# caidj0/Raytracer-2025

Measured on NVIDIA B200. Metric: paths_per_sec, higher is better.
Workload: dtype f64

## Files before the change

raytracer-2025_b200/csrc/api.cu:

```cuda
#include <cuda_runtime.h>

#include <algorithm>
#include <cstdio>
#include <cstdlib>
#include <cstring>
#include <memory>
#include <mutex>
#include <new>
#include <string>
#include <thread>
#include <vector>

#include "compile.h"
#include "kernels.h"
#include "rt2025.h"

using namespace rt;

namespace {

thread_local std::string g_err;

int set_err(int code, const std::string& msg) {
    g_err = msg;
// ... 247 lines not shown
        if (rc != RT_OK) return set_err(rc, err);
        if (!device_build) {
            rc = check_device(opts ? opts->device : -1, device, sms);
            if (rc != RT_OK) return rc;
        }
        {
            const size_t budget = EXTEND_SMEM_MAX / EXTEND_MIN_BLOCKS - 1024;
            const size_t stacks = (size_t)std::min<uint32_t>(std::max(cs.bvh_depth + 2, 3 * cs.bvh4_depth + 2), TRAVERSAL_STACK) * EXTEND_BLOCK * sizeof(uint32_t) + EXTEND_RAY_SMEM_BYTES;
            if (!cs.nodes4.empty() && cs.nodes.size() * sizeof(Node) <= 2 * budget && stacks + cs.nodes4.size() * sizeof(Node4) > budget &&
                !getenv("RT2025_WIDE_BVH")) {
                RawVec<Node4>().swap(cs.nodes4);
                cs.world_root4 = INVALID_REF;
            }
        }
        s = new rt_scene();
        s->device = device;
        s->sm_count = sms;
        SceneView& v = s->view;
        keep_pool_memory(device);
        {
            cudaStream_t st = cudaStreamPerThread;
            Arena a;
            a.reserve(cs.nodes4), a.reserve(cs.nodes), a.reserve(cs.geom), a.reserve(cs.meta), a.reserve(cs.xforms), a.reserve(cs.materials), a.reserve(cs.textures);
            a.reserve(cs.images), a.reserve(cs.texels), a.reserve(cs.perlins), a.reserve(cs.media), a.reserve(cs.lights), a.reserve(cs.remaps), a.reserve(cs.walk_lean);
            a.allocate(st);
            s->arena = a.base;
            v.nodes4 = a.put(cs.nodes4, st), v.world_root4 = cs.world_root4;
            v.nodes = a.put(cs.nodes, st), v.geom = a.put(cs.geom, st), v.meta = a.put(cs.meta, st), v.xforms = a.put(cs.xforms, st);
            v.materials = a.put(cs.materials, st), v.textures = a.put(cs.textures, st), v.images = a.put(cs.images, st);
            v.texels = a.put(cs.texels, st), v.perlins = a.put(cs.perlins, st), v.media = a.put(cs.media, st);
            v.lights = a.put(cs.lights, st), v.remaps = a.put(cs.remaps, st), v.walk_lean = a.put(cs.walk_lean, st);
            CU(cudaStreamSynchronize(st));
        }
        v.world_root = cs.world_root;
        v.n_media = (uint32_t)cs.media.size();
        v.n_xforms = (uint32_t)cs.xforms.size();
        v.kinds = (cs.n_spheres && !cs.n_planars) ? 1u : ((cs.n_planars && !cs.n_spheres) ? 2u : 0u);
        v.n_lights = (uint32_t)cs.lights.size();
        v.n_prims = (uint32_t)cs.geom.size();
        s->ranks = cs.ranks;
        for (auto& m : cs.media) s->generic_media |= m.single_sphere == RT_NONE;
        v.media_xform = 0;
        for (auto& m : cs.media)
            if (m.xform != RT_NONE || (m.single_sphere != RT_NONE && cs.meta[m.single_sphere].xform != RT_NONE)) v.media_xform = 1;
        for (auto& m : cs.materials) s->class_mask |= 1u << m.shade_class;
        for (auto& t : cs.textures) s->black_texture.push_back(t.kind == RT_TEX_SOLID && t.color[0] == 0.0 && t.color[1] == 0.0 && t.color[2] == 0.0);
        uint32_t n_thick = 0, n_thick_entries = 0;
        for (auto& m : cs.media)
            if (m.flags & MEDIUM_THICK) s->class_mask |= 1u << SC_WALK, n_thick++, n_thick_entries += m.n_entry != MEDIUM_NO_ENTRIES;
        v.walk_entries_only = n_thick == 1 && n_thick_entries == 1;
        s->lights_flat = 1;
        for (auto& l : cs.lights)
            if (l.weight != 1.0 / (double)cs.lights.size()) s->lights_flat = 0;
        rt_scene_info& i = s->info;
// ... 362 lines not shown
                    cudaEventDestroy(ws.events.back());
                    ws.events.pop_back();
                }
            }
        }
        launch_finalize(W.accum, n_px_img * 3, cam->pixel_sample_scale, d_accum, o.accum_type == RT_ACCUM_F64, grid_g, st);
        launches += 1;
        CU(cudaEventRecord(ev[1], st));
        CU(cudaEventSynchronize(ev[1]));
        CU(cudaGetLastError());
        if (stats) {
            float ms = 0;
            CU(cudaEventElapsedTime(&ms, ev[0], ev[1]));
            const Counters zero{};
            const Counters& c = final_counters ? *final_counters : zero;
            stats->paths = nominal_paths;
            stats->segments = total_paths ? c.segments : 0;
            stats->node_visits = total_paths ? c.node_visits : 0;
            stats->prim_tests = total_paths ? c.prim_tests : 0;
            stats->errors = total_paths ? c.errors : 0;
            stats->iterations = total_paths ? c.iterations : 0;
            stats->reserved[0] = total_paths ? c.walk_segments : 0;
            stats->reserved[1] = total_paths ? c.walk_lean_segments : 0;
            stats->kernel_launches = launches;
            stats->ms_total = ms;
            stats->ms_raygen = ms_gen, stats->ms_extend = ms_ext, stats->ms_shade = ms_shd;
            stats->ms_other = ms_med;
        }
    } catch (const CudaFail& f) {
        rc = set_err(RT_ERR_CUDA, f.what);
    }
    for (auto& e : ev)
        if (e) cudaEventDestroy(e);
    return rc;
}

int rt_render(const rt_scene* s, const rt_camera* cam, const rt_render_opts* opts, void* accum, rt_stats* stats) {
    if (!s || !cam || !accum) return set_err(RT_ERR_INVALID, "null argument");
    const size_t elem = (opts && opts->accum_type == RT_ACCUM_F64) ? 8 : 4;
    const size_t bytes = (size_t)cam->image_width * cam->image_height * 3 * elem;
    void* d = nullptr;
    int rc = RT_OK;
    DeviceGuard guard;
    try {
        CU(cudaSetDevice(s->device));
        scratch_alloc(&d, bytes);
// ... 264 lines not shown
```

raytracer-2025_b200/csrc/compile.cpp:

```cpp
#include "compile.h"

#include <omp.h>

#include <memory>
#include <parallel/algorithm>

#include <chrono>
#include <cstdio>
#include <cstdlib>

#include <vector_functions.h>

#include <algorithm>
#include <cmath>
#include <cstring>
#include <limits>

namespace rt {

namespace {

struct V3 {
    double x, y, z;
};
// ... 962 lines not shown
            med.flags = 0;
            if (!all_spheres || !(min_depth > 0.0)) continue;
            const double radius = std::fabs(out.geom[med.single_sphere].d[6]);
            if (radius * std::fabs(1.0 / med.neg_inv_density) >= min_depth) med.flags |= MEDIUM_THICK;
        }
        for (size_t m = 0; m < out.media.size(); m++) {
            Medium& med = out.media[m];
            med.n_entry = MEDIUM_NO_ENTRIES;
            if (!(med.flags & MEDIUM_THICK) || getenv("RT2025_WALK_NO_ENTRIES")) continue;
            GroupBox b = group_boxes[group_of_medium[m]];
            for (int k = 0; k < 3; k++) {
                const float pad = 1e-4f * std::max(1.0f, std::max(std::fabs(b.lo[k]), std::fabs(b.hi[k])));
                b.lo[k] -= pad, b.hi[k] += pad;
            }
            uint32_t n = 0;
            const double* g = out.geom[med.single_sphere].d;
            const bool plain = med.xform == RT_NONE && out.meta[med.single_sphere].xform == RT_NONE && g[3] == 0.0 && g[4] == 0.0 && g[5] == 0.0;
            const double ball[4] = {g[0], g[1], g[2], std::fabs(g[6]) * (1.0 + 1e-4) + 1e-4};
            if (overlapping_leaves(b, plain ? ball : nullptr, out.world_root, med.entry, n)) med.n_entry = n;
            if (timer.on) fprintf(stderr, "[rt2025 compile] medium %zu is optically thick: %d entry leaves\n", m, (int)med.n_entry);
        }
        walk_lean();
        if (timer.on) fprintf(stderr, "[rt2025 compile] random walk: %s\n", out.walk_lean.empty() ? "generic" : (out.walk_lean[0].shell != RT_NONE ? "lean, shell" : "lean"));
        return RT_OK;
    }

    void walk_lean() {
        out.walk_lean.clear();
        const size_t n_media = out.media.size(), n_lights = out.lights.size();
        if (n_media > WALK_LEAN_MEDIA || n_lights > WALK_LEAN_LIGHTS) return;
        WalkLean L;
        std::memset(&L, 0, sizeof(L));
        L.n_media = (uint32_t)n_media, L.n_lights = (uint32_t)n_lights, L.thick = RT_NONE, L.shell = RT_NONE;
        for (size_t m = 0; m < n_media; m++) {
            const Medium& med = out.media[m];
            if (med.single_sphere == RT_NONE || med.xform != RT_NONE || out.meta[med.single_sphere].xform != RT_NONE) return;
            if (med.flags & MEDIUM_THICK) {
                if (L.thick != RT_NONE || med.n_entry == MEDIUM_NO_ENTRIES) return;
                L.thick = (uint32_t)m;
            }
            std::memcpy(L.sphere[m], out.geom[med.single_sphere].d, 7 * sizeof(double));
            L.neg_inv_density[m] = med.neg_inv_density;
            L.rank[m] = med.rank, L.medium_index[m] = med.medium_index;
        }
        if (L.thick == RT_NONE) return;
        const Medium& thick = out.media[L.thick];
        const Material& iso = out.materials[thick.material];
        if (iso.kind != RT_MAT_ISOTROPIC || iso.tex >= out.textures.size() || out.textures[iso.tex].kind != RT_TEX_SOLID) return;
        for (int k = 0; k < 3; k++) L.axp[k] = (1.0 / (4.0 * 3.14159265358979323846264338327950288)) * out.textures[iso.tex].color[k];
        for (size_t i = 0; i < n_lights; i++) {
            const Light& l = out.lights[i];
            if (l.xform != RT_NONE || l.weight != 1.0 / (double)n_lights) return;
            L.lights[i] = l;
        }
        for (uint32_t e = 0; e < thick.n_entry; e++) {
            const uint32_t first = (thick.entry[e] & ~LEAF_FLAG) >> 3, count = (thick.entry[e] & 7u) + 1;
            for (uint32_t pi = first; pi < first + count; pi++) {
                const PrimMeta& pm = out.meta[pi];
                if (L.n_prims == WALK_LEAN_PRIMS || pm.xform != RT_NONE) return;
                const uint32_t k = L.n_prims++;
                L.prim[k] = out.geom[pi];
                L.prim_kind[k] = pm.kind_mat >> 30, L.prim_rank[k] = pm.rank;
                if (L.shell == RT_NONE && L.prim_kind[k] == PRIM_SPHERE && std::memcmp(out.geom[pi].d, L.sphere[L.thick], 7 * sizeof(double)) == 0) L.shell = k;
            }
        }
        out.walk_lean.push_back(L);
    }
};

}

int compile_scene(const rt_scene_desc& d, uint32_t flags, CompiledScene& out, std::string& err, WorldBuilder world_builder) {
    Compiler c{d, flags, out, err};
    c.world_builder = world_builder;
    return c.run();
}

}
```

raytracer-2025_b200/csrc/compile.h:

```cpp
#pragma once
#include <memory>
#include <string>
#include <type_traits>
#include <utility>
#include <vector>

#include <vector_types.h>

#include "rt2025.h"
#include "scene_types.h"

namespace rt {

template <class T, class A = std::allocator<T>>
struct default_init_allocator : A {
    using A::A;
    template <class U>
    struct rebind {
        using other = default_init_allocator<U, typename std::allocator_traits<A>::template rebind_alloc<U>>;
    };
    template <class U>
    void construct(U* p) noexcept(std::is_nothrow_default_constructible<U>::value) {
        ::new (static_cast<void*>(p)) U;
    }
// ... 3 lines not shown
    }
};
template <class T>
using RawVec = std::vector<T, default_init_allocator<T>>;

struct CompiledScene {
    RawVec<Node> nodes;
    RawVec<Node4> nodes4;
    uint32_t world_root4 = INVALID_REF;
    uint32_t bvh4_depth = 0;
    RawVec<PrimGeom> geom;
    RawVec<PrimMeta> meta;
    std::vector<Xform> xforms;
    std::vector<Material> materials;
    std::vector<Texture> textures;
    std::vector<Image> images;
    std::vector<float4> texels;
    std::vector<Perlin> perlins;
    std::vector<Medium> media;
    std::vector<Light> lights;
    std::vector<Remap> remaps;
    std::vector<uint32_t> ranks;
    std::vector<WalkLean> walk_lean;
    uint32_t world_root = INVALID_REF;
    uint32_t bvh_depth = 0;
    uint32_t media_bvh_depth = 0;
    uint32_t n_spheres = 0, n_planars = 0;
};

struct BuildBox;
using WorldBuilder = bool (*)(const RawVec<BuildBox>& boxes, uint32_t first_prim_base, RawVec<Node>& nodes,
                              RawVec<uint32_t>& order, uint32_t& depth_out, uint32_t& root_out);

int compile_scene(const rt_scene_desc& d, uint32_t flags, CompiledScene& out, std::string& err, WorldBuilder world_builder = nullptr);

uint32_t collapse_bvh4(const RawVec<Node>& nodes, uint32_t root, RawVec<Node4>& out, uint32_t& depth_out);

struct BuildBox {
    float lo[3], hi[3];
};
uint32_t build_bvh(const RawVec<BuildBox>& boxes, uint32_t first_prim_base, RawVec<Node>& nodes,
                   RawVec<uint32_t>& order, uint32_t& depth_out);
bool build_bvh_device(const RawVec<BuildBox>& boxes, uint32_t first_prim_base, RawVec<Node>& nodes, RawVec<uint32_t>& order,
                      uint32_t& depth_out, uint32_t& root_out);

}
// ... 1 lines not shown
```

raytracer-2025_b200/csrc/kernels.cu:

```cuda
#include <cuda_runtime.h>
#include <stdint.h>

#include <algorithm>

#include "kernels.h"
#include "shade.cuh"

namespace rt {

struct RayArrayIO {
    const SceneView& sv;
    const rt_ray* __restrict__ rays;
    rt_hit* __restrict__ out;
    double tmin, tmax;
    __device__ __forceinline__ double t_min() const { return tmin; }
    __device__ __forceinline__ bool load(uint32_t i, RayD& r, double& t1, uint32_t& prim0, uint32_t& rank0) const {
        const double* rp = reinterpret_cast<const double*>(rays + i);
        r.o = D3{rp[0], rp[1], rp[2]};
        r.d = D3{rp[3], rp[4], rp[5]};
        r.time = rp[6];
        t1 = tmax;
        prim0 = 0xFFFFFFFFu, rank0 = 0xFFFFFFFFu;
        return true;
    }
// ... 469 lines not shown
        const uint32_t local = queue_reserve(cntb, q);
        __syncthreads();
        if (threadIdx.x < SC_COUNT) {
            const uint32_t c = cntb[threadIdx.x];
            if (c) s_base[threadIdx.x] = atomicAdd(&W.counters->n_shade[threadIdx.x], c);
            s_cnt[(it & 1) ^ 1][threadIdx.x] = 0;
        }
        __syncthreads();
        if (q >= 0) W.q_shade[q][s_base[q] + local] = j;
    }
}

__device__ __forceinline__ void contribute(const RenderParams& P, const WavefrontState& W, uint32_t pixel, D3 c) {
    if (isnan(c.x) || isnan(c.y) || isnan(c.z)) {
        atomicAdd(&W.counters->errors, 1ull);
        return;
    }
    double* a = W.accum + (size_t)pixel * 3;
    if (c.x != 0.0) atomicAdd(a + 0, c.x);
    if (c.y != 0.0) atomicAdd(a + 1, c.y);
    if (c.z != 0.0) atomicAdd(a + 2, c.z);
}

template <uint32_t CLS>
__device__ __forceinline__ bool shade_one(const SceneView& sv, const RenderParams& P, const WavefrontState& W, const RayD& r, D3 beta, uint32_t pixel,
                                          uint32_t sidx, uint32_t segment, double t, uint32_t prim, uint32_t kind, RayD& nr, D3& nbeta) {
    constexpr bool GENERIC = CLS == SC_OTHER;
    constexpr bool DO_MISS = CLS == SC_MISS;
    constexpr bool DO_MEDIUM = GENERIC || CLS == SC_ISOTROPIC;
    constexpr bool DO_EMIT = GENERIC || CLS == SC_EMISSIVE || CLS == SC_DISNEY;
    constexpr bool DO_PDF = GENERIC || CLS == SC_DIFFUSE || CLS == SC_TEXTURED || CLS == SC_ISOTROPIC || CLS == SC_DISNEY;
    constexpr bool DO_REMAP = GENERIC || CLS == SC_DISNEY;
    constexpr bool DO_METAL = GENERIC || CLS == SC_METAL;
    constexpr bool DO_DIELECTRIC = GENERIC || CLS == SC_DIELECTRIC;
            bool alive = false, error = false;
            nr = r;
            nbeta = beta;

            if (DO_MISS || (GENERIC && kind == HIT_MISS)) {
                D3 bg;
                if (background_value(sv, P.cam.background_tex, r.d, bg))
                    contribute(P, W, pixel, beta * bg);
                else
                    error = true;
            } else {
                HitInfo h;
                bool hit_ok = true;
                if (DO_MEDIUM && kind == HIT_MEDIUM) {
                    const Medium& med = sv.media[prim];
// ... 82 lines not shown
                        }
                        case RT_MAT_TRANSPARENT:
                            alive = GENERIC;
                            break;
                        case RT_MAT_PORTAL: {
                            if (!GENERIC) break;
                            nr.o = h.p + ld3(M.v);
                            double qw = M.v[3], qx = M.v[4], qy = M.v[5], qz = M.v[6];
                            double aw = qw * 0.0 - qx * r.d.x - qy * r.d.y - qz * r.d.z;
                            double ax = qw * r.d.x + qx * 0.0 + qy * r.d.z - qz * r.d.y;
                            double ay = qw * r.d.y - qx * r.d.z + qy * 0.0 + qz * r.d.x;
                            double az = qw * r.d.z + qx * r.d.y - qy * r.d.x + qz * 0.0;
                            double cx = -qx, cy = -qy, cz = -qz;
                            nr.d.x = aw * cx + ax * qw + ay * cz - az * cy;
                            nr.d.y = aw * cy - ax * cz + ay * qw + az * cx;
                            nr.d.z = aw * cz + ax * cy - ay * cx + az * qw;
                            nbeta = beta * ld3(M.color);
                            alive = true;
                            break;
                        }
                        case RT_MAT_LAMBERTIAN: {
                            const bool iso = CLS == SC_ISOTROPIC || (GENERIC && M.kind == RT_MAT_ISOTROPIC);
                            const bool dis = CLS == SC_DISNEY || (GENERIC && M.kind == RT_MAT_DISNEY);
                            D3 albedo = (M.kind == RT_MAT_EMPTY || dis) ? D3{0.75, 0.75, 0.75} : texture_value(sv, M.tex, h.u, h.v, h.p);
                            ONB uvw;
                            if (!iso && !make_onb(h.normal, uvw)) {
                                error = true;
                                break;
                            }
                            disney::Params DP;
                            D3 v_out_l = D3{0.0, 1.0, 0.0};
                            if (dis) {
                                DP.base_color = M.tex == RT_NONE ? ld3(M.color) : texture_value(sv, M.tex, h.u, h.v, h.p);
                                DP.roughness = M.v[RT_DISNEY_ROUGHNESS], DP.anisotropic = M.v[RT_DISNEY_ANISOTROPIC], DP.sheen = M.v[RT_DISNEY_SHEEN];
                                DP.sheen_tint = M.v[RT_DISNEY_SHEEN_TINT], DP.clearcoat = M.v[RT_DISNEY_CLEARCOAT];
                                DP.clearcoat_gloss = M.v[RT_DISNEY_CLEARCOAT_GLOSS], DP.specular_tint = M.v[RT_DISNEY_SPECULAR_TINT];
                                DP.metallic = M.v[RT_DISNEY_METALLIC], DP.ior = M.v[RT_DISNEY_IOR], DP.flatness = M.v[RT_DISNEY_FLATNESS];
                                DP.spec_trans = M.v[RT_DISNEY_SPEC_TRANS], DP.diff_trans = M.v[RT_DISNEY_DIFF_TRANS], DP.thin = M.v[RT_DISNEY_THIN] != 0.0;
                                D3 vo;
                                if (!unit_vector(-r.d, vo)) {
                                    error = true;
                                    break;
                                }
                                v_out_l = D3{dot(vo, uvw.u), dot(vo, uvw.v), dot(vo, uvw.w)};
                            }
                            Rand2 pick = philox_pair(P.seed, pixel, sidx, segment, RT_SLOT_MIXTURE);
                            Rand2 dx = philox_pair(P.seed, pixel, sidx, segment, RT_SLOT_DIRECTION);
                            D3 gen = D3{0.0, 0.0, 0.0};
                            const bool have_lights = sv.n_lights > 0;
                            int stop = 0;
                            if (have_lights && !(pick.a < 0.5)) {
                                if (!lights_random(sv, h.p, pick.b, dx.a, dx.b, gen)) stop = 1;
                            } else if (dis) {
                                Rand2 dpick = philox_pair(P.seed, pixel, sidx, segment, RT_SLOT_DISNEY);
                                D3 v_in_l;
                                bool derr = false;
                                if (!disney::generate_local(DP, v_out_l, h.front_face, dpick, dx, v_in_l, derr))
                                    stop = derr ? 1 : 2;
                                else if (!unit_vector(onb_to_world(uvw, v_in_l), gen))
                                    stop = 1;
                            } else {
                                gen = iso ? random_unit_vector(dx.a, dx.b) : onb_to_world(uvw, random_cosine_direction(dx.a, dx.b));
                            }
                            D3 axp = D3{0.0, 0.0, 0.0};
                            double value0 = 0.0;
                            if (!stop) {
                                if (iso) {
                                    value0 = 1.0 / (4.0 * RT_PI);
                                    axp = albedo / (4.0 * RT_PI);
                                } else {
                                    D3 ud;
                                    if (!unit_vector(gen, ud)) {
                                        stop = 1;
                                    } else if (dis) {
                                        D3 v_in_l = D3{dot(ud, uvw.u), dot(ud, uvw.v), dot(ud, uvw.w)};
                                        bool derr = false;
                                        disney::evaluate_disney(DP, v_out_l, v_in_l, h.front_face, axp, value0, derr);
                                        if (derr) stop = 1;
                                    } else {
                                        double cosine_theta = dot(ud, uvw.v);
                                        value0 = rmax(0.0, cosine_theta / RT_PI);
                                        axp = albedo * rmax(cosine_theta, 0.0) / RT_PI;
                                    }
                                }
                            }
                            double pdf_val = value0;
                            if (!stop && have_lights) {
                                double value1 = lights_pdf_value(sv, P.lights_flat, h.p, gen);
                                if (isnan(value1) || (value0 == 0.0 && value1 == 0.0))
                                    stop = 1;
                                else
                                    pdf_val = value0 * 0.5 + value1 * 0.5;
                            }
                            if (!stop && pdf_val == 0.0) stop = 1;
                            if (!stop) {
                                nr.d = gen;
                                nbeta = beta * (axp / pdf_val);
                                alive = true;
                            }
                            if (stop == 1) error = true;
                            break;
                        }
                        default: break;
                    }
                }
            }
            if (error) {
                atomicAdd(&W.counters->errors, 1ull);
                alive = false;
            }
            if (alive && (segment + 1 >= P.cam.max_depth || (nbeta.x == 0.0 && nbeta.y == 0.0 && nbeta.z == 0.0))) alive = false;
            return alive;
}

template <uint32_t CLS>
__global__ void __launch_bounds__(SHADE_BLOCK, ((RT_SHADE_3BLOCK_MASK >> CLS) & 1u) ? 3 : RT_SHADE_MIN_BLOCKS) k_shade(SceneView sv, RenderParams P, WavefrontState W, uint32_t queue) {
    __shared__ uint32_t s_warp_count[SHADE_BLOCK / 32];
    __shared__ uint32_t s_base;
    const uint32_t n = W.counters->n_shade[queue];
    const RayRec* __restrict__ rays = W.ray_q[W.parity];
    const BetaRec* __restrict__ betas = W.beta_q[W.parity];
    for (uint32_t j0 = blockIdx.x * blockDim.x; j0 < n; j0 += gridDim.x * blockDim.x) {
        const uint32_t j = j0 + threadIdx.x;
        int q = -1;
        RayD nr;
        D3 nbeta;
        uint32_t pixel = 0, sidx = 0, segment = 0;
#if RT_SHADE_PREFETCH
        {
            const uint32_t jn = j + gridDim.x * blockDim.x;
            if (jn < n) {
                const uint32_t pn = W.q_shade[queue][jn];
                asm volatile("prefetch.global.L2 [%0];" ::"l"(rays + pn));
                asm volatile("prefetch.global.L2 [%0];" ::"l"(betas + pn));
                asm volatile("prefetch.global.L2 [%0];" ::"l"(W.hit_q + pn));
            }
        }
#endif
        if (j < n) {
            const uint32_t pos = W.q_shade[queue][j];
            RayD r;
            uint64_t ids64;
            load_ray(rays + pos, r, ids64);
            unpack_ids(ids64, pixel, sidx, segment);
            const double2* sp2 = reinterpret_cast<const double2*>(betas + pos);
            const double2 b0 = sp2[0], b1 = sp2[1];
            D3 beta = D3{b0.x, b0.y, b1.x};
            const double2 hw = *reinterpret_cast<const double2*>(W.hit_q + pos);
            const double t = hw.x;
            const uint32_t prim = (uint32_t)__double2hiint(hw.y), kind = (uint32_t)__double2loint(hw.y);
            const bool alive = shade_one<CLS>(sv, P, W, r, beta, pixel, sidx, segment, t, prim, kind, nr, nbeta);
            q = alive ? 0 : -1;
        }
        const unsigned alive_mask = __ballot_sync(0xFFFFFFFFu, q == 0);
        const uint32_t warp = threadIdx.x >> 5, lane = threadIdx.x & 31u;
        if (lane == 0) s_warp_count[warp] = __popc(alive_mask);
        __syncthreads();
        if (threadIdx.x == 0) {
            uint32_t total = 0;
#pragma unroll
            for (int w = 0; w < SHADE_BLOCK / 32; w++) total += s_warp_count[w];
            s_base = total ? atomicAdd(&W.counters->n_extend[W.parity ^ 1u], total) : 0u;
        }
        __syncthreads();
        uint32_t npos = s_base + __popc(alive_mask & ((1u << lane) - 1u));
        for (uint32_t w = 0; w < warp; w++) npos += s_warp_count[w];
        __syncthreads();
        if (q == 0) {
            store_ray(W.ray_q[W.parity ^ 1u] + npos, nr, pack_ids(pixel, sidx, segment + 1));
            store_beta(W.beta_q[W.parity ^ 1u] + npos, nbeta);
        }
    }
}

#ifndef RT_WALK_BLOCK
#define RT_WALK_BLOCK 128
#endif
constexpr int WALK_BLOCK = RT_WALK_BLOCK;
#ifndef RT_WALK_MIN_BLOCKS
#define RT_WALK_MIN_BLOCKS 4
#endif
#ifndef RT_WALK_LEAN_MIN_BLOCKS
#define RT_WALK_LEAN_MIN_BLOCKS 4
#endif

__device__ __forceinline__ bool walk_lean_segment(const SceneView& sv, const WalkLean& L, const RenderParams& P, const WavefrontState& W, const RayD& r,
                                                  D3 beta, uint32_t pixel, uint32_t sidx, uint32_t segment, double t, uint32_t max_steps,
                                                  uint32_t& steps, RayD& nr, D3& nbeta, double& tn, bool& stay) {
    stay = false;
    nr.o = r.o + t * r.d;
    nr.time = r.time;
    const Rand2 pick = philox_pair(P.seed, pixel, sidx, segment, RT_SLOT_MIXTURE);
    const Rand2 dx = philox_pair(P.seed, pixel, sidx, segment, RT_SLOT_DIRECTION);
    const uint32_t n_lights = L.n_lights;
    D3 gen = D3{0.0, 0.0, 0.0};
    bool panic = false;
    if (n_lights > 0 && !(pick.a < 0.5)) {
        uint32_t leaf = n_lights - 1;
        for (uint32_t i = 0; i < n_lights; i++)
            if (pick.b < L.lights[i].cdf) {
                leaf = i;
                break;
            }
        panic = !light_leaf_random(L.lights[leaf], nr.o, dx.a, dx.b, gen);
    } else {
        gen = random_unit_vector(dx.a, dx.b);
    }
    const double value0 = 1.0 / (4.0 * RT_PI);
    double pdf_val = value0;
    if (!panic && n_lights > 0) {
        double sum = 0.0;
        for (uint32_t i = 0; i < n_lights; i++) sum += light_leaf_pdf<true>(sv, L.lights[i], nr.o, gen);
        const double value1 = n_lights == 1 ? sum : sum / (double)n_lights;
        if (isnan(value1) || (value0 == 0.0 && value1 == 0.0))
            panic = true;
        else
            pdf_val = value0 * 0.5 + value1 * 0.5;
    }
    if (panic || pdf_val == 0.0) {
        atomicAdd(&W.counters->errors, 1ull);
        return false;
    }
    nr.d = gen;
    nbeta = beta * (ld3(L.axp) / pdf_val);
    if (segment + 1 >= P.cam.max_depth || (nbeta.x == 0.0 && nbeta.y == 0.0 && nbeta.z == 0.0)) return false;

    const uint32_t seg1 = segment + 1u, thick = L.thick;
    MediumDraws draws;
    double near_root, far_root;
    {
        const double* s = L.sphere[thick];
        double t1, t2;
        const double xi = draws.get(P.seed, pixel, sidx, seg1, L.medium_index[thick]);
        const bool inside = sphere_entry_exit_at(ld3(s), ld3(s + 3), s[6], nr, t1, t2, near_root, far_root);
        if (!inside || !medium_free_flight(t1, t2, nr, L.neg_inv_density[thick], xi, tn)) return true;
    }
    if (!(++steps < max_steps)) return true;
    const uint32_t med_rank = L.rank[thick];
    for (uint32_t m = 0; m < L.n_media; m++) {
        if (m == thick) continue;
        const double xi = draws.get(P.seed, pixel, sidx, seg1, L.medium_index[m]);
        if (RT_MEDIA_EARLY_SCREEN && free_flight_overshoots(L.neg_inv_density[m], xi, tn, nr.d)) continue;
        const double* s = L.sphere[m];
        double t1, t2, nroot, froot, tm;
        if (!sphere_entry_exit_at(ld3(s), ld3(s + 3), s[6], nr, t1, t2, nroot, froot) || !medium_free_flight(t1, t2, nr, L.neg_inv_density[m], xi, tm)) continue;
        if (tm < tn || (tm == tn && L.rank[m] < med_rank)) return true;
    }
    bool beaten = false;
// ... 297 lines not shown
        k<<<grid, MEDIA_BLOCK, 0, s>>>(sv, P, W);
        return 1;
    }
    int launches = 1;
    if (phase == 0 && sv.n_media) {
        SceneView mv = sv;
        mv.n_cached_nodes = 0;
        const size_t media_smem = generic ? (size_t)sv.media_stack_entries * MEDIA_BLOCK * sizeof(uint32_t) : 0;
        const bool xf = sv.media_xform != 0;
        if (generic) {
            auto k = count ? (xf ? k_media<true, 2, true, false> : k_media<true, 2, false, false>) : (xf ? k_media<false, 2, true, false> : k_media<false, 2, false, false>);
            k<<<grid, MEDIA_BLOCK, media_smem, s>>>(mv, P, W);
        } else {
            auto k = count ? (xf ? k_media<true, 1, true, false> : k_media<true, 1, false, false>) : (xf ? k_media<false, 1, true, false> : k_media<false, 1, false, false>);
            k<<<grid, MEDIA_BLOCK, 0, s>>>(mv, P, W);
        }
        launches++;
    }
    k_bin<<<grid, MEDIA_BLOCK, 0, s>>>(W);
    return launches;
}
template <uint32_t CLS>
static void launch_shade_cls(const SceneView& sv, const RenderParams& P, const WavefrontState& W, uint32_t queue, int grid, cudaStream_t s) {
    if ((RT_SHADE_3BLOCK_MASK >> CLS) & 1u) grid = grid / RT_SHADE_MIN_BLOCKS * 3;
    k_shade<CLS><<<grid, SHADE_BLOCK, 0, s>>>(sv, P, W, queue);
}
int launch_shade(const SceneView& sv, const RenderParams& P, const WavefrontState& W, uint32_t class_mask, int grid, cudaStream_t s,
                 const ShadeFan* fan, bool tail_follows, int walk_grid) {
    int launches = tail_follows ? 1 : 2;
    if (!P.bin_by_class) {
        launch_shade_cls<SC_MISS>(sv, P, W, SC_MISS, grid, s);
        launch_shade_cls<SC_OTHER>(sv, P, W, SC_DIFFUSE, grid, s);
        launches++;
    } else {
        const int n_side = fan ? fan->n_side : 0;
        if (n_side) {
            cudaEventRecord(fan->fork, s);
            for (int i = 0; i < n_side; i++) cudaStreamWaitEvent(fan->side[i], fan->fork, 0);
        }
        int next = 0;
        auto lane = [&]() {
            const int k = next++ % (n_side + 1);
            return k == 0 ? s : fan->side[k - 1];
        };
        if (class_mask & (1u << SC_WALK)) launch_walk(sv, P, W, walk_grid, lane()), launches++;
        if (class_mask & (1u << SC_DIFFUSE)) launch_shade_cls<SC_DIFFUSE>(sv, P, W, SC_DIFFUSE, grid, lane()), launches++;
// ... 53 lines not shown
```

raytracer-2025_b200/csrc/kernels.h:

```cpp
#pragma once
#include <cuda_runtime.h>
#include <stdint.h>

#include "rt2025.h"
#include "scene_types.h"

namespace rt {

#ifndef RT_EXTEND_BLOCK
#define RT_EXTEND_BLOCK 512
#endif
#ifndef RT_EXTEND_MIN_BLOCKS
#define RT_EXTEND_MIN_BLOCKS 1
#endif
constexpr int EXTEND_BLOCK = RT_EXTEND_BLOCK;
constexpr int EXTEND_MIN_BLOCKS = RT_EXTEND_MIN_BLOCKS;
constexpr size_t EXTEND_SMEM_MAX = 227 * 1024;
constexpr int SHADE_BLOCK = 256;
constexpr int MEDIA_BLOCK = 256;
#ifndef RT_REFILL_MIN
#define RT_REFILL_MIN 32
#endif
constexpr int REFILL_MIN = RT_REFILL_MIN;
#ifndef RT_SLAB_SIGNSEL
// ... 47 lines not shown
    double w[7];
    uint64_t ids;
};
struct alignas(16) BetaRec {
    double beta[3];
    double spare;
};
struct alignas(16) HitRec {
    double t;
    uint32_t kind, prim;
};
static_assert(sizeof(RayRec) == 64 && sizeof(BetaRec) == 32 && sizeof(HitRec) == 16, "stream record sizes");
constexpr uint32_t IDS_PIXEL_BITS = 28, IDS_SAMPLE_BITS = 24, IDS_SEGMENT_BITS = 12;

struct Counters {
    uint32_t n_extend[2];
    uint32_t n_shade[SC_COUNT];
    uint32_t n_pixels, pad;
    uint32_t n_unsampled, pad3;
    uint32_t gen_done, walk_cursor;
    unsigned long long next_path, segments, iterations, errors, node_visits, prim_tests;
    unsigned long long walk_segments;
    unsigned long long walk_lean_segments;
};

struct WavefrontState {
    RayRec* ray_q[2];
    BetaRec* beta_q[2];
    HitRec* hit_q;
    uint8_t* cls_q;
    uint32_t* q_shade[SC_COUNT];
    uint32_t* pixel_list;
    double* accum;
    Counters* counters;
    uint32_t capacity, n_pixels;
    uint64_t total_paths;
    uint32_t parity, pad;
};

struct RenderParams {
    rt_camera cam;
    uint64_t seed;
    uint32_t sample_begin, part_index, part_count;
    uint32_t lights_flat, bin_by_class;
    uint32_t walk_drain_queue, walk_drain_steps;
    uint32_t drop_misses;
// ... 30 lines not shown
```

raytracer-2025_b200/csrc/scene_types.h:

```cpp
#pragma once
#include <stdint.h>

namespace rt {

constexpr uint32_t LEAF_FLAG = 0x80000000u;
constexpr uint32_t INVALID_REF = 0x7FFFFFFFu;
constexpr int MAX_LEAF_PRIMS = 8;
constexpr int TRAVERSAL_STACK = 64;
constexpr uint32_t META_MAT_MASK = 0x03FFFFFFu;
constexpr uint32_t META_CLASS_SHIFT = 26;

struct alignas(32) Node {
    float lo0[3], hi0[3];
    float lo1[3], hi1[3];
    uint32_t child0, child1;
    uint32_t pad0, pad1;
};
static_assert(sizeof(Node) == 64, "node must be 64 bytes");

struct alignas(32) Node4 {
    float box[4][6];
    uint32_t child[4];
    uint32_t pad[4];
};
// ... 59 lines not shown
struct Medium {
    uint32_t root;
    uint32_t material;
    uint32_t object;
    uint32_t rank;
    double neg_inv_density;
    uint32_t xform;
    uint32_t medium_index;
    uint32_t single_sphere;
    uint32_t flags;
    uint32_t n_entry;
    uint32_t entry[MEDIUM_MAX_ENTRIES];
    uint32_t pad;
};
constexpr uint32_t MEDIUM_THICK = 1u;

struct Light {
    PrimGeom g;
    uint32_t kind;
    uint32_t xform;
    double weight, cdf, area;
};

constexpr uint32_t WALK_LEAN_MEDIA = 4, WALK_LEAN_LIGHTS = 4, WALK_LEAN_PRIMS = 8;
struct WalkLean {
    Light lights[WALK_LEAN_LIGHTS];
    PrimGeom prim[WALK_LEAN_PRIMS];
    double sphere[WALK_LEAN_MEDIA][8];
    double neg_inv_density[WALK_LEAN_MEDIA];
    double axp[3];
    double pad0;
    uint32_t rank[WALK_LEAN_MEDIA], medium_index[WALK_LEAN_MEDIA];
    uint32_t prim_kind[WALK_LEAN_PRIMS], prim_rank[WALK_LEAN_PRIMS];
    uint32_t n_media, thick, n_lights, n_prims;
    uint32_t shell;
    uint32_t pad1[3];
};

enum ShadeClass : uint32_t {
    SC_MISS = 0,
    SC_DIFFUSE = 1,
    SC_TEXTURED = 2,
    SC_ISOTROPIC = 3,
    SC_METAL = 4,
    SC_DIELECTRIC = 5,
    SC_EMISSIVE = 6,
    SC_DISNEY = 7,
    SC_OTHER = 8,
    SC_WALK = 9,
    SC_COUNT = 10
};

struct SceneView {
    const Node* nodes;
    const PrimGeom* geom;
    const PrimMeta* meta;
    const Xform* xforms;
    const Material* materials;
    const Texture* textures;
// ... 1 lines not shown
    const float4* texels;
    const Perlin* perlins;
    const Medium* media;
    const Light* lights;
    const Remap* remaps;
    const Node4* nodes4;
    uint32_t world_root4;
    uint32_t media_xform;
    uint32_t world_root;
    uint32_t n_media, n_lights, n_prims;
    uint32_t n_nodes;
    uint32_t n_cached_nodes;
    uint32_t stack_entries;
    uint32_t l2_window_bytes;
    uint32_t park_leaves;
    uint32_t refill_min;
    uint32_t media_stack_entries;
    uint32_t tail_stack_entries;
    uint32_t kinds;
    uint32_t n_xforms;
    uint32_t walk_entries_only;
    uint32_t fifo_slots;
    const WalkLean* walk_lean;
};

}
```

raytracer-2025_b200/csrc/shade.cuh:

```cuda
#pragma once
#include "disney.cuh"
#include "traverse.cuh"

namespace rt {

__device__ __forceinline__ int32_t as_i32_sat(double x) {
    if (isnan(x)) return 0;
    if (x >= 2147483647.0) return 2147483647;
    if (x <= -2147483648.0) return (-2147483647 - 1);
    return (int32_t)x;
}
__device__ __forceinline__ uint32_t as_u32_sat(double x) {
    if (!(x > 0.0)) return 0u;
    if (x >= 4294967295.0) return 0xFFFFFFFFu;
    return (uint32_t)x;
}

__device__ inline double perlin_noise(const Perlin* __restrict__ tab, D3 p) {
    double fx = floor(p.x), fy = floor(p.y), fz = floor(p.z);
    long long i = (long long)fx, j = (long long)fy, k = (long long)fz;
    double u = p.x - fx, v = p.y - fy, w = p.z - fz;
    double uu = u * u * (3.0 - 2.0 * u), vv = v * v * (3.0 - 2.0 * v), ww = w * w * (3.0 - 2.0 * w);
    double accum = 0.0;
#pragma unroll
// ... 240 lines not shown
    for (uint32_t i = 0; i < sv.n_lights; i++)
        if (pick < sv.lights[i].cdf) {
            leaf = i;
            break;
        }
    const Light& l = sv.lights[leaf];
    if (l.xform == RT_NONE) return light_leaf_random(l, origin, r1, r2, out);
    const Xform* x = sv.xforms + l.xform;
    const uint32_t n = x->n_chain;
    D3 origins[MAX_XFORM_CHAIN + 1];
    origins[0] = origin;
    for (uint32_t k = 0; k < n; k++) origins[k + 1] = xf_detransform(load_xform(sv.xforms + x->chain[k]), origins[k]);
    D3 dir;
    bool ok = light_leaf_random(l, origins[n], r1, r2, dir);
    for (uint32_t k = n; k-- > 0;) {
        XformParams p = load_xform(sv.xforms + x->chain[k]);
        D3 world_to = xf_transform(p, origins[k + 1] + dir);
        ok = unit_vector(world_to - origins[k], dir) && ok;
    }
    out = dir;
    return ok;
}

__device__ inline bool background_value(const SceneView& sv, uint32_t tex, D3 dir, D3& out) {
    D3 p;
    if (!unit_vector(dir, p)) return false;
    double u = 0.0, v = 0.0;
    if (texture_needs_uv(sv, tex)) {
        double theta = acos(-p.y);
        double phi = RT_PI - atan2(-p.z, p.x);
        u = phi / (2.0 * RT_PI);
        v = theta / RT_PI;
    }
    out = texture_value(sv, tex, u, v, p);
    return true;
}

__device__ inline D3 material_emitted(const SceneView& sv, uint32_t mat, const HitInfo& h) {
    D3 total = D3{0.0, 0.0, 0.0};
    uint32_t st_mat[8];
    double st_w[8];
    int sp = 0;
    st_mat[sp] = mat, st_w[sp] = 1.0, sp++;
    while (sp > 0) {
        --sp;
        uint32_t m = st_mat[sp];
// ... 20 lines not shown
```

raytracer-2025_b200/rt2025.py:

```python
import ctypes as C
import os
import subprocess

import numpy as np

PKG_DIR = os.path.dirname(os.path.abspath(__file__))
ROOT = os.path.dirname(PKG_DIR)
RT_NONE = 0xFFFFFFFF
RT_OPT_COUNT = 1
RT_OPT_STAGE_TIMES = 2
RT_ACCUM_F32 = 0
RT_ACCUM_F64 = 1
RT_BUILD_NO_REF_RANKS = 1
RT_BUILD_DEVICE_LBVH = 2

ABI_SYMBOLS = [
    "rt_scene_create", "rt_scene_destroy", "rt_closest_hit", "rt_closest_hit_device", "rt_render",
    "rt_render_device", "rt_render_rgb8", "rt_render_multi", "rt_render_multi_rgb8", "rt_tonemap", "rt_tonemap_device", "rt_scene_get_info", "rt_scene_get_ranks", "rt_last_error",
    "rt_abi_version", "rt_device_count",
]


class RtError(RuntimeError):
    pass
# ... 23 lines not shown
        ("reserved", C.c_uint32 * 4),
    ]


class rt_stats(C.Structure):
    _fields_ = [
        ("paths", C.c_uint64), ("segments", C.c_uint64), ("node_visits", C.c_uint64),
        ("prim_tests", C.c_uint64), ("errors", C.c_uint64), ("kernel_launches", C.c_uint64),
        ("ms_total", C.c_double), ("ms_raygen", C.c_double), ("ms_extend", C.c_double),
        ("ms_shade", C.c_double), ("ms_other", C.c_double), ("iterations", C.c_uint64),
        ("reserved", C.c_uint64 * 4),
    ]

    def as_dict(self):
        return {k: getattr(self, k) for k, _ in self._fields_ if k != "reserved"}

    @property
    def walk_segments(self):
        return int(self.reserved[0])

    @property
    def walk_lean_segments(self):
        return int(self.reserved[1])


class rt_scene_info(C.Structure):
    _fields_ = [
        ("n_prims", C.c_uint32), ("n_spheres", C.c_uint32), ("n_planars", C.c_uint32), ("n_nodes", C.c_uint32),
        ("n_media", C.c_uint32), ("n_lights", C.c_uint32), ("n_materials", C.c_uint32), ("n_textures", C.c_uint32),
        ("bvh_depth", C.c_uint32), ("node_bytes", C.c_uint32), ("device_bytes", C.c_uint64),
    ]


class rth_camera_params(C.Structure):
    _fields_ = [
        ("aspect_ratio", C.c_double), ("image_width", C.c_uint32), ("samples_per_pixel", C.c_uint32),
        ("max_depth", C.c_uint32), ("background_tex", C.c_uint32), ("vertical_fov_in_degrees", C.c_double),
        ("look_from", C.c_double * 3), ("look_at", C.c_double * 3), ("vec_up", C.c_double * 3),
        ("defocus_angle_in_degrees", C.c_double), ("focus_distance", C.c_double),
        ("toon_map", C.c_uint32), ("reserved", C.c_uint32),
    ]


class rt_scene_desc(C.Structure):
    _fields_ = [
        ("version", C.c_uint32), ("struct_size", C.c_uint32), ("world_root", C.c_uint32), ("lights_root", C.c_uint32),
# ... 388 lines not shown
```

Before: 1.509 billion.

## Add lean specialized shade kernels for diffuse, textured, isotropic and emissive classes

After: 1.586 billion, median of 6. 5.2% higher.

```diff
diff --git a/raytracer-2025_b200/csrc/api.cu b/raytracer-2025_b200/csrc/api.cu
--- a/raytracer-2025_b200/csrc/api.cu
+++ b/raytracer-2025_b200/csrc/api.cu
@@ -293,7 +293,7 @@
             cudaStream_t st = cudaStreamPerThread;
             Arena a;
             a.reserve(cs.nodes4), a.reserve(cs.nodes), a.reserve(cs.geom), a.reserve(cs.meta), a.reserve(cs.xforms), a.reserve(cs.materials), a.reserve(cs.textures);
-            a.reserve(cs.images), a.reserve(cs.texels), a.reserve(cs.perlins), a.reserve(cs.media), a.reserve(cs.lights), a.reserve(cs.remaps), a.reserve(cs.walk_lean);
+            a.reserve(cs.images), a.reserve(cs.texels), a.reserve(cs.perlins), a.reserve(cs.media), a.reserve(cs.lights), a.reserve(cs.remaps), a.reserve(cs.walk_lean), a.reserve(cs.shade_lean);
             a.allocate(st);
             s->arena = a.base;
             v.nodes4 = a.put(cs.nodes4, st), v.world_root4 = cs.world_root4;
@@ -301,6 +301,7 @@
             v.materials = a.put(cs.materials, st), v.textures = a.put(cs.textures, st), v.images = a.put(cs.images, st);
             v.texels = a.put(cs.texels, st), v.perlins = a.put(cs.perlins, st), v.media = a.put(cs.media, st);
             v.lights = a.put(cs.lights, st), v.remaps = a.put(cs.remaps, st), v.walk_lean = a.put(cs.walk_lean, st);
+            v.shade_lean = a.put(cs.shade_lean, st), v.shade_lean_mask = cs.shade_lean_mask;
             CU(cudaStreamSynchronize(st));
         }
         v.world_root = cs.world_root;
@@ -709,6 +710,7 @@
             stats->iterations = total_paths ? c.iterations : 0;
             stats->reserved[0] = total_paths ? c.walk_segments : 0;
             stats->reserved[1] = total_paths ? c.walk_lean_segments : 0;
+            stats->reserved[2] = total_paths ? c.shade_lean_hits : 0;
             stats->kernel_launches = launches;
             stats->ms_total = ms;
             stats->ms_raygen = ms_gen, stats->ms_extend = ms_ext, stats->ms_shade = ms_shd;
diff --git a/raytracer-2025_b200/csrc/compile.cpp b/raytracer-2025_b200/csrc/compile.cpp
--- a/raytracer-2025_b200/csrc/compile.cpp
+++ b/raytracer-2025_b200/csrc/compile.cpp
@@ -1008,16 +1008,45 @@
         }
         walk_lean();
         if (timer.on) fprintf(stderr, "[rt2025 compile] random walk: %s\n", out.walk_lean.empty() ? "generic" : (out.walk_lean[0].shell != RT_NONE ? "lean, shell" : "lean"));
+        shade_lean();
+        if (timer.on) {
+            std::string classes;
+            const std::pair<uint32_t, const char*> names[] = {{SC_DIFFUSE, " diffuse"}, {SC_TEXTURED, " textured"}, {SC_ISOTROPIC, " isotropic"}, {SC_EMISSIVE, " emissive"}};
+            for (const auto& c : names)
+                if (out.shade_lean_mask & (1u << c.first)) classes += c.second;
+            fprintf(stderr, "[rt2025 compile] shade lean:%s\n", classes.empty() ? " generic" : classes.c_str());
+        }
         return RT_OK;
+    }
+
+    bool lean_lights(LeanLights& L) const {
+        std::memset(&L, 0, sizeof(L));
+        const size_t n = out.lights.size();
+        if (n > LEAN_LIGHTS) return false;
+        for (size_t i = 0; i < n; i++) {
+            const Light& l = out.lights[i];
+            if (l.xform != RT_NONE || l.weight != 1.0 / (double)n) return false;
+            L.lights[i] = l;
+        }
+        L.n = (uint32_t)n;
+        return true;
+    }
+
+    bool isotropic_axp(uint32_t material, double* axp) const {
+        const Material& iso = out.materials[material];
+        if (iso.kind != RT_MAT_ISOTROPIC || iso.tex >= out.textures.size() || out.textures[iso.tex].kind != RT_TEX_SOLID) return false;
+        for (int k = 0; k < 3; k++) axp[k] = (1.0 / (4.0 * 3.14159265358979323846264338327950288)) * out.textures[iso.tex].color[k];
+        return true;
     }
 
     void walk_lean() {
         out.walk_lean.clear();
-        const size_t n_media = out.media.size(), n_lights = out.lights.size();
-        if (n_media > WALK_LEAN_MEDIA || n_lights > WALK_LEAN_LIGHTS) return;
+        const size_t n_media = out.media.size();
+        if (n_media > WALK_LEAN_MEDIA) return;
         WalkLean L;
         std::memset(&L, 0, sizeof(L));
-        L.n_media = (uint32_t)n_media, L.n_lights = (uint32_t)n_lights, L.thick = RT_NONE, L.shell = RT_NONE;
+        if (!lean_lights(L.lights)) return;
+        L.n_media = (uint32_t)n_media, L.thick = RT_NONE, L.shell = RT_NONE;
         for (size_t m = 0; m < n_media; m++) {
             const Medium& med = out.media[m];
             if (med.single_sphere == RT_NONE || med.xform != RT_NONE || out.meta[med.single_sphere].xform != RT_NONE) return;
@@ -1031,14 +1060,7 @@
         }
         if (L.thick == RT_NONE) return;
         const Medium& thick = out.media[L.thick];
-        const Material& iso = out.materials[thick.material];
-        if (iso.kind != RT_MAT_ISOTROPIC || iso.tex >= out.textures.size() || out.textures[iso.tex].kind != RT_TEX_SOLID) return;
-        for (int k = 0; k < 3; k++) L.axp[k] = (1.0 / (4.0 * 3.14159265358979323846264338327950288)) * out.textures[iso.tex].color[k];
-        for (size_t i = 0; i < n_lights; i++) {
-            const Light& l = out.lights[i];
-            if (l.xform != RT_NONE || l.weight != 1.0 / (double)n_lights) return;
-            L.lights[i] = l;
-        }
+        if (!isotropic_axp(thick.material, L.axp)) return;
         for (uint32_t e = 0; e < thick.n_entry; e++) {
             const uint32_t first = (thick.entry[e] & ~LEAF_FLAG) >> 3, count = (thick.entry[e] & 7u) + 1;
             for (uint32_t pi = first; pi < first + count; pi++) {
@@ -1052,6 +1074,36 @@
         }
         out.walk_lean.push_back(L);
     }
+
+    void shade_lean() {
+        out.shade_lean.clear();
+        out.shade_lean_mask = 0;
+        ShadeLean S;
+        std::memset(&S, 0, sizeof(S));
+        const bool lights = lean_lights(S.lights);
+        bool iso = lights && out.media.size() <= SHADE_LEAN_MEDIA;
+        for (size_t m = 0; iso && m < out.media.size(); m++) {
+            const Medium& med = out.media[m];
+            if (med.flags & MEDIUM_THICK) continue;
+            iso = med.xform == RT_NONE && isotropic_axp(med.material, S.axp[m]);
+        }
+        bool emissive = true;
+        for (size_t p = 0; p < out.meta.size() && (iso || emissive); p++) {
+            const PrimMeta& pm = out.meta[p];
+            const uint32_t cls = (pm.kind_mat >> META_CLASS_SHIFT) & 15u;
+            if (cls == SC_ISOTROPIC) iso = false;
+            if (cls == SC_EMISSIVE) {
+                const Material& M = out.materials[pm.kind_mat & META_MAT_MASK];
+                if (pm.xform != RT_NONE || M.kind != RT_MAT_DIFFUSE_LIGHT || M.inner != RT_NONE || M.tex >= out.textures.size() ||
+                    out.textures[M.tex].kind != RT_TEX_SOLID)
+                    emissive = false;
+            }
+        }
+        if (lights) out.shade_lean_mask |= 1u << SC_DIFFUSE | 1u << SC_TEXTURED;
+        if (iso) out.shade_lean_mask |= 1u << SC_ISOTROPIC;
+        if (emissive) out.shade_lean_mask |= 1u << SC_EMISSIVE;
+        if (out.shade_lean_mask) out.shade_lean.push_back(S);
+    }
 };
 
 }
diff --git a/raytracer-2025_b200/csrc/compile.h b/raytracer-2025_b200/csrc/compile.h
--- a/raytracer-2025_b200/csrc/compile.h
+++ b/raytracer-2025_b200/csrc/compile.h
@@ -49,6 +49,8 @@
     std::vector<Remap> remaps;
     std::vector<uint32_t> ranks;
     std::vector<WalkLean> walk_lean;
+    std::vector<ShadeLean> shade_lean;
+    uint32_t shade_lean_mask = 0;
     uint32_t world_root = INVALID_REF;
     uint32_t bvh_depth = 0;
     uint32_t media_bvh_depth = 0;
diff --git a/raytracer-2025_b200/csrc/kernels.cu b/raytracer-2025_b200/csrc/kernels.cu
--- a/raytracer-2025_b200/csrc/kernels.cu
+++ b/raytracer-2025_b200/csrc/kernels.cu
@@ -515,9 +515,11 @@
     if (c.z != 0.0) atomicAdd(a + 2, c.z);
 }
 
-template <uint32_t CLS>
+template <uint32_t CLS, bool LEAN = false>
 __device__ __forceinline__ bool shade_one(const SceneView& sv, const RenderParams& P, const WavefrontState& W, const RayD& r, D3 beta, uint32_t pixel,
-                                          uint32_t sidx, uint32_t segment, double t, uint32_t prim, uint32_t kind, RayD& nr, D3& nbeta) {
+                                          uint32_t sidx, uint32_t segment, double t, uint32_t prim, uint32_t kind, RayD& nr, D3& nbeta,
+                                          const LeanLights* LL = nullptr) {
+    static_assert(!LEAN || CLS == SC_DIFFUSE || CLS == SC_TEXTURED, "the other lean classes have their own code");
     constexpr bool GENERIC = CLS == SC_OTHER;
     constexpr bool DO_MISS = CLS == SC_MISS;
     constexpr bool DO_MEDIUM = GENERIC || CLS == SC_ISOTROPIC;
@@ -646,7 +648,9 @@
                         case RT_MAT_LAMBERTIAN: {
                             const bool iso = CLS == SC_ISOTROPIC || (GENERIC && M.kind == RT_MAT_ISOTROPIC);
                             const bool dis = CLS == SC_DISNEY || (GENERIC && M.kind == RT_MAT_DISNEY);
-                            D3 albedo = (M.kind == RT_MAT_EMPTY || dis) ? D3{0.75, 0.75, 0.75} : texture_value(sv, M.tex, h.u, h.v, h.p);
+                            D3 albedo = (M.kind == RT_MAT_EMPTY || dis)  ? D3{0.75, 0.75, 0.75}
+                                        : (LEAN && CLS == SC_DIFFUSE) ? ld3(sv.textures[M.tex].color)
+                                                                      : texture_value(sv, M.tex, h.u, h.v, h.p);
                             ONB uvw;
                             if (!iso && !make_onb(h.normal, uvw)) {
                                 error = true;
@@ -671,10 +675,10 @@
                             Rand2 pick = philox_pair(P.seed, pixel, sidx, segment, RT_SLOT_MIXTURE);
                             Rand2 dx = philox_pair(P.seed, pixel, sidx, segment, RT_SLOT_DIRECTION);
                             D3 gen = D3{0.0, 0.0, 0.0};
-                            const bool have_lights = sv.n_lights > 0;
+                            const bool have_lights = LEAN ? LL->n > 0 : sv.n_lights > 0;
                             int stop = 0;
                             if (have_lights && !(pick.a < 0.5)) {
-                                if (!lights_random(sv, h.p, pick.b, dx.a, dx.b, gen)) stop = 1;
+                                if (!(LEAN ? lean_lights_random(*LL, h.p, pick.b, dx.a, dx.b, gen) : lights_random(sv, h.p, pick.b, dx.a, dx.b, gen))) stop = 1;
                             } else if (dis) {
                                 Rand2 dpick = philox_pair(P.seed, pixel, sidx, segment, RT_SLOT_DISNEY);
                                 D3 v_in_l;
@@ -710,7 +714,7 @@
                             }
                             double pdf_val = value0;
                             if (!stop && have_lights) {
-                                double value1 = lights_pdf_value(sv, P.lights_flat, h.p, gen);
+                                double value1 = LEAN ? lean_lights_pdf(sv, *LL, h.p, gen) : lights_pdf_value(sv, P.lights_flat, h.p, gen);
                                 if (isnan(value1) || (value0 == 0.0 && value1 == 0.0))
                                     stop = 1;
                                 else
@@ -737,10 +741,59 @@
             return alive;
 }
 
-template <uint32_t CLS>
-__global__ void __launch_bounds__(SHADE_BLOCK, ((RT_SHADE_3BLOCK_MASK >> CLS) & 1u) ? 3 : RT_SHADE_MIN_BLOCKS) k_shade(SceneView sv, RenderParams P, WavefrontState W, uint32_t queue) {
+__device__ __forceinline__ bool lean_isotropic_scatter(const SceneView& sv, const LeanLights& L, D3 axp, const RenderParams& P, const WavefrontState& W,
+                                                       const RayD& r, D3 beta, uint32_t pixel, uint32_t sidx, uint32_t segment, double t, RayD& nr,
+                                                       D3& nbeta) {
+    nr.o = r.o + t * r.d;
+    nr.time = r.time;
+    const Rand2 pick = philox_pair(P.seed, pixel, sidx, segment, RT_SLOT_MIXTURE);
+    const Rand2 dx = philox_pair(P.seed, pixel, sidx, segment, RT_SLOT_DIRECTION);
+    D3 gen = D3{0.0, 0.0, 0.0};
+    bool panic = false;
+    if (L.n > 0 && !(pick.a < 0.5))
+        panic = !lean_lights_random(L, nr.o, pick.b, dx.a, dx.b, gen);
+    else
+        gen = random_unit_vector(dx.a, dx.b);
+    const double value0 = 1.0 / (4.0 * RT_PI);
+    double pdf_val = value0;
+    if (!panic && L.n > 0) {
+        const double value1 = lean_lights_pdf(sv, L, nr.o, gen);
+        if (isnan(value1) || (value0 == 0.0 && value1 == 0.0))
+            panic = true;
+        else
+            pdf_val = value0 * 0.5 + value1 * 0.5;
+    }
+    if (panic || pdf_val == 0.0) {
+        atomicAdd(&W.counters->errors, 1ull);
+        return false;
+    }
+    nr.d = gen;
+    nbeta = beta * (axp / pdf_val);
+    return !(segment + 1 >= P.cam.max_depth || (nbeta.x == 0.0 && nbeta.y == 0.0 && nbeta.z == 0.0));
+}
+
+#ifndef RT_SHADE_LEAN_BLOCKS
+#define RT_SHADE_LEAN_BLOCKS 0x3003230u
+#endif
+constexpr int shade_lean_blocks(uint32_t cls) { return (int)((RT_SHADE_LEAN_BLOCKS >> (4u * cls)) & 15u); }
+constexpr int shade_blocks(uint32_t cls, bool lean) {
+    return lean ? shade_lean_blocks(cls) : (((RT_SHADE_3BLOCK_MASK >> cls) & 1u) ? 3 : RT_SHADE_MIN_BLOCKS);
+}
+
+template <uint32_t CLS, bool LEAN = false>
+__global__ void __launch_bounds__(SHADE_BLOCK, shade_blocks(CLS, LEAN)) k_shade(SceneView sv, RenderParams P, WavefrontState W, uint32_t queue) {
+    constexpr bool EMIT_ONLY = LEAN && CLS == SC_EMISSIVE;
     __shared__ uint32_t s_warp_count[SHADE_BLOCK / 32];
     __shared__ uint32_t s_base;
+    extern __shared__ float4 s_lean[];
+    const ShadeLean& SL = *reinterpret_cast<const ShadeLean*>(s_lean);
+    if (LEAN && !EMIT_ONLY) {
+        unsigned long long* dst = reinterpret_cast<unsigned long long*>(s_lean);
+        const unsigned long long* src = reinterpret_cast<const unsigned long long*>(sv.shade_lean);
+        for (uint32_t k = threadIdx.x; k < sizeof(ShadeLean) / 8; k += SHADE_BLOCK) dst[k] = src[k];
+        __syncthreads();
+    }
+    unsigned long long lean_hits = 0;
     const uint32_t n = W.counters->n_shade[queue];
     const RayRec* __restrict__ rays = W.ray_q[W.parity];
     const BetaRec* __restrict__ betas = W.beta_q[W.parity];
@@ -761,21 +814,38 @@
             }
         }
 #endif
+        if (LEAN && threadIdx.x == 0) lean_hits += min(n - j0, (uint32_t)SHADE_BLOCK);
         if (j < n) {
             const uint32_t pos = W.q_shade[queue][j];
-            RayD r;
-            uint64_t ids64;
-            load_ray(rays + pos, r, ids64);
-            unpack_ids(ids64, pixel, sidx, segment);
-            const double2* sp2 = reinterpret_cast<const double2*>(betas + pos);
-            const double2 b0 = sp2[0], b1 = sp2[1];
-            D3 beta = D3{b0.x, b0.y, b1.x};
-            const double2 hw = *reinterpret_cast<const double2*>(W.hit_q + pos);
-            const double t = hw.x;
-            const uint32_t prim = (uint32_t)__double2hiint(hw.y), kind = (uint32_t)__double2loint(hw.y);
-            const bool alive = shade_one<CLS>(sv, P, W, r, beta, pixel, sidx, segment, t, prim, kind, nr, nbeta);
-            q = alive ? 0 : -1;
-        }
+            if constexpr (EMIT_ONLY) {
+                unpack_ids((uint64_t)__double_as_longlong(reinterpret_cast<const double2*>(rays + pos)[3].y), pixel, sidx, segment);
+                const double2* sp2 = reinterpret_cast<const double2*>(betas + pos);
+                const double2 b0 = sp2[0], b1 = sp2[1];
+                const D3 beta = D3{b0.x, b0.y, b1.x};
+                const uint32_t prim = (uint32_t)__double2hiint(reinterpret_cast<const double2*>(W.hit_q + pos)->y);
+                const uint32_t mat = sv.meta[prim].kind_mat & META_MAT_MASK;
+                const D3 e = D3{0.0, 0.0, 0.0} + 1.0 * ld3(sv.textures[sv.materials[mat].tex].color);
+                contribute(P, W, pixel, beta * e);
+            } else {
+                RayD r;
+                uint64_t ids64;
+                load_ray(rays + pos, r, ids64);
+                unpack_ids(ids64, pixel, sidx, segment);
+                const double2* sp2 = reinterpret_cast<const double2*>(betas + pos);
+                const double2 b0 = sp2[0], b1 = sp2[1];
+                D3 beta = D3{b0.x, b0.y, b1.x};
+                const double2 hw = *reinterpret_cast<const double2*>(W.hit_q + pos);
+                const double t = hw.x;
+                const uint32_t prim = (uint32_t)__double2hiint(hw.y), kind = (uint32_t)__double2loint(hw.y);
+                bool alive;
+                if constexpr (LEAN && CLS == SC_ISOTROPIC)
+                    alive = lean_isotropic_scatter(sv, SL.lights, ld3(SL.axp[prim]), P, W, r, beta, pixel, sidx, segment, t, nr, nbeta);
+                else
+                    alive = shade_one<CLS, LEAN>(sv, P, W, r, beta, pixel, sidx, segment, t, prim, kind, nr, nbeta, &SL.lights);
+                q = alive ? 0 : -1;
+            }
+        }
+        if constexpr (EMIT_ONLY) continue;
         const unsigned alive_mask = __ballot_sync(0xFFFFFFFFu, q == 0);
         const uint32_t warp = threadIdx.x >> 5, lane = threadIdx.x & 31u;
         if (lane == 0) s_warp_count[warp] = __popc(alive_mask);
@@ -790,11 +860,14 @@
         uint32_t npos = s_base + __popc(alive_mask & ((1u << lane) - 1u));
         for (uint32_t w = 0; w < warp; w++) npos += s_warp_count[w];
         __syncthreads();
-        if (q == 0) {
-            store_ray(W.ray_q[W.parity ^ 1u] + npos, nr, pack_ids(pixel, sidx, segment + 1));
-            store_beta(W.beta_q[W.parity ^ 1u] + npos, nbeta);
-        }
-    }
+        if constexpr (!EMIT_ONLY) {
+            if (q == 0) {
+                store_ray(W.ray_q[W.parity ^ 1u] + npos, nr, pack_ids(pixel, sidx, segment + 1));
+                store_beta(W.beta_q[W.parity ^ 1u] + npos, nbeta);
+            }
+        }
+    }
+    if (LEAN && lean_hits) atomicAdd(&W.counters->shade_lean_hits, lean_hits);
 }
 
 #ifndef RT_WALK_BLOCK
@@ -812,42 +885,7 @@
                                                   D3 beta, uint32_t pixel, uint32_t sidx, uint32_t segment, double t, uint32_t max_steps,
                                                   uint32_t& steps, RayD& nr, D3& nbeta, double& tn, bool& stay) {
     stay = false;
-    nr.o = r.o + t * r.d;
-    nr.time = r.time;
-    const Rand2 pick = philox_pair(P.seed, pixel, sidx, segment, RT_SLOT_MIXTURE);
-    const Rand2 dx = philox_pair(P.seed, pixel, sidx, segment, RT_SLOT_DIRECTION);
-    const uint32_t n_lights = L.n_lights;
-    D3 gen = D3{0.0, 0.0, 0.0};
-    bool panic = false;
-    if (n_lights > 0 && !(pick.a < 0.5)) {
-        uint32_t leaf = n_lights - 1;
-        for (uint32_t i = 0; i < n_lights; i++)
-            if (pick.b < L.lights[i].cdf) {
-                leaf = i;
-                break;
-            }
-        panic = !light_leaf_random(L.lights[leaf], nr.o, dx.a, dx.b, gen);
-    } else {
-        gen = random_unit_vector(dx.a, dx.b);
-    }
-    const double value0 = 1.0 / (4.0 * RT_PI);
-    double pdf_val = value0;
-    if (!panic && n_lights > 0) {
-        double sum = 0.0;
-        for (uint32_t i = 0; i < n_lights; i++) sum += light_leaf_pdf<true>(sv, L.lights[i], nr.o, gen);
-        const double value1 = n_lights == 1 ? sum : sum / (double)n_lights;
-        if (isnan(value1) || (value0 == 0.0 && value1 == 0.0))
-            panic = true;
-        else
-            pdf_val = value0 * 0.5 + value1 * 0.5;
-    }
-    if (panic || pdf_val == 0.0) {
-        atomicAdd(&W.counters->errors, 1ull);
-        return false;
-    }
-    nr.d = gen;
-    nbeta = beta * (ld3(L.axp) / pdf_val);
-    if (segment + 1 >= P.cam.max_depth || (nbeta.x == 0.0 && nbeta.y == 0.0 && nbeta.z == 0.0)) return false;
+    if (!lean_isotropic_scatter(sv, L.lights, ld3(L.axp), P, W, r, beta, pixel, sidx, segment, t, nr, nbeta)) return false;
 
     const uint32_t seg1 = segment + 1u, thick = L.thick;
     MediumDraws draws;
@@ -1191,6 +1229,13 @@
 }
 template <uint32_t CLS>
 static void launch_shade_cls(const SceneView& sv, const RenderParams& P, const WavefrontState& W, uint32_t queue, int grid, cudaStream_t s) {
+    if constexpr (CLS == SC_DIFFUSE || CLS == SC_TEXTURED || CLS == SC_ISOTROPIC || CLS == SC_EMISSIVE) {
+        if (queue == CLS && (sv.shade_lean_mask >> CLS) & 1u) {
+            static_assert(shade_lean_blocks(CLS) >= 1, "RT_SHADE_LEAN_BLOCKS: no CTA count for a lean class");
+            k_shade<CLS, true><<<grid / RT_SHADE_MIN_BLOCKS * shade_lean_blocks(CLS), SHADE_BLOCK, CLS == SC_EMISSIVE ? 0 : sizeof(ShadeLean), s>>>(sv, P, W, queue);
+            return;
+        }
+    }
     if ((RT_SHADE_3BLOCK_MASK >> CLS) & 1u) grid = grid / RT_SHADE_MIN_BLOCKS * 3;
     k_shade<CLS><<<grid, SHADE_BLOCK, 0, s>>>(sv, P, W, queue);
 }
diff --git a/raytracer-2025_b200/csrc/kernels.h b/raytracer-2025_b200/csrc/kernels.h
--- a/raytracer-2025_b200/csrc/kernels.h
+++ b/raytracer-2025_b200/csrc/kernels.h
@@ -93,6 +93,7 @@
     unsigned long long next_path, segments, iterations, errors, node_visits, prim_tests;
     unsigned long long walk_segments;
     unsigned long long walk_lean_segments;
+    unsigned long long shade_lean_hits;
 };
 
 struct WavefrontState {
diff --git a/raytracer-2025_b200/csrc/scene_types.h b/raytracer-2025_b200/csrc/scene_types.h
--- a/raytracer-2025_b200/csrc/scene_types.h
+++ b/raytracer-2025_b200/csrc/scene_types.h
@@ -105,9 +105,16 @@
     double weight, cdf, area;
 };
 
-constexpr uint32_t WALK_LEAN_MEDIA = 4, WALK_LEAN_LIGHTS = 4, WALK_LEAN_PRIMS = 8;
+constexpr uint32_t LEAN_LIGHTS = 4;
+struct LeanLights {
+    Light lights[LEAN_LIGHTS];
+    uint32_t n;
+    uint32_t pad[7];
+};
+
+constexpr uint32_t WALK_LEAN_MEDIA = 4, WALK_LEAN_PRIMS = 8;
 struct WalkLean {
-    Light lights[WALK_LEAN_LIGHTS];
+    LeanLights lights;
     PrimGeom prim[WALK_LEAN_PRIMS];
     double sphere[WALK_LEAN_MEDIA][8];
     double neg_inv_density[WALK_LEAN_MEDIA];
@@ -115,9 +122,14 @@
     double pad0;
     uint32_t rank[WALK_LEAN_MEDIA], medium_index[WALK_LEAN_MEDIA];
     uint32_t prim_kind[WALK_LEAN_PRIMS], prim_rank[WALK_LEAN_PRIMS];
-    uint32_t n_media, thick, n_lights, n_prims;
+    uint32_t n_media, thick, n_prims;
     uint32_t shell;
-    uint32_t pad1[3];
+};
+
+constexpr uint32_t SHADE_LEAN_MEDIA = 4;
+struct ShadeLean {
+    LeanLights lights;
+    double axp[SHADE_LEAN_MEDIA][4];
 };
 
 enum ShadeClass : uint32_t {
@@ -165,6 +177,8 @@
     uint32_t walk_entries_only;
     uint32_t fifo_slots;
     const WalkLean* walk_lean;
+    const ShadeLean* shade_lean;
+    uint32_t shade_lean_mask;
 };
 
 }
diff --git a/raytracer-2025_b200/csrc/shade.cuh b/raytracer-2025_b200/csrc/shade.cuh
--- a/raytracer-2025_b200/csrc/shade.cuh
+++ b/raytracer-2025_b200/csrc/shade.cuh
@@ -286,6 +286,21 @@
     return ok;
 }
 
+__device__ __forceinline__ bool lean_lights_random(const LeanLights& L, D3 origin, double pick, double r1, double r2, D3& out) {
+    uint32_t leaf = L.n - 1;
+    for (uint32_t i = 0; i < L.n; i++)
+        if (pick < L.lights[i].cdf) {
+            leaf = i;
+            break;
+        }
+    return light_leaf_random(L.lights[leaf], origin, r1, r2, out);
+}
+__device__ __forceinline__ double lean_lights_pdf(const SceneView& sv, const LeanLights& L, D3 origin, D3 direction) {
+    double sum = 0.0;
+    for (uint32_t i = 0; i < L.n; i++) sum += light_leaf_pdf<true>(sv, L.lights[i], origin, direction);
+    return L.n == 1 ? sum : sum / (double)L.n;
+}
+
 __device__ inline bool background_value(const SceneView& sv, uint32_t tex, D3 dir, D3& out) {
     D3 p;
     if (!unit_vector(dir, p)) return false;
diff --git a/raytracer-2025_b200/rt2025.py b/raytracer-2025_b200/rt2025.py
--- a/raytracer-2025_b200/rt2025.py
+++ b/raytracer-2025_b200/rt2025.py
@@ -69,6 +69,10 @@
     @property
     def walk_lean_segments(self):
         return int(self.reserved[1])
+
+    @property
+    def shade_lean_hits(self):
+        return int(self.reserved[2])
 
 
 class rt_scene_info(C.Structure):
```
